# hongsukchoi/Pose2Mesh_RELEASE

Hardware: NVIDIA H100
Metric: SMPL meshes/sec (higher is better)
Workload: dtype f32 (wgmma fp16x3 split, fp32 accumulate)

## Files before the change

include/p2m_b200.h:

```cpp
#ifndef P2M_B200_H_
#define P2M_B200_H_

#include <stddef.h>
#include <stdint.h>

#ifdef __cplusplus
extern "C" {
#endif

typedef struct p2m_model p2m_model_t;
typedef void* p2m_stream_t;

enum p2m_status {
  P2M_OK = 0,
  P2M_ERR_INVALID = 1,
  P2M_ERR_CUDA = 2,
  P2M_ERR_WORKSPACE = 3,
  P2M_ERR_NOGPU = 4
};

enum p2m_precision {
  P2M_PREC_FP32_SIMT = 0,
  P2M_PREC_FP16X3_TC = 1
};
// ... 23 lines not shown
} p2m_params_t;

int p2m_model_create(const p2m_model_desc_t* desc, p2m_model_t** out);
void p2m_model_destroy(p2m_model_t* m);
int p2m_model_num_layers(const p2m_model_t* m);
int p2m_model_layer_info(const p2m_model_t* m, int layer, int32_t out[6]);
int p2m_model_set_precision(p2m_model_t* m, int precision);
int p2m_model_set_profiling(p2m_model_t* m, int enable);
int p2m_model_layer_times_ms(p2m_model_t* m, float* out_ms, int n);
int p2m_debug_kernel_status(p2m_model_t* m, int32_t* out);
int p2m_debug_set_trace(p2m_model_t* m, void* dev_buf);
int p2m_debug_set_fuse_head(p2m_model_t* m, int enable);
int p2m_debug_set_elide_padding(p2m_model_t* m, int enable);
int p2m_debug_set_dedup_padding(p2m_model_t* m, int enable);
int p2m_debug_conv_path(const p2m_model_t* m, int level, int fin, int fout, int32_t out[9]);
int p2m_debug_layer_route(const p2m_model_t* m, int layer, int batch, int need_dx, int32_t out[9]);

typedef struct {
  float* const* z;
  float* const* a;
  float* const* y;
  float* fc_out;
  float* const* g_a;
  float* const* g_z;
  float* const* dx;
  float* fc_dx;
} p2m_capture_t;
int p2m_debug_set_capture(p2m_model_t* m, const p2m_capture_t* capture);

#define P2M_BN_BATCH_UPDATE 0
// ... 350 lines not shown
```

pose2mesh_release_b200/_lib.py:

```python
from __future__ import annotations

import ctypes as C
import os
import threading

import torch

_HERE = os.path.dirname(os.path.abspath(__file__))
LIB_PATH = os.path.join(_HERE, "libp2m_b200.so")

P2M_PREC_FP32_SIMT = 0
P2M_PREC_FP16X3_TC = 1
PRECISIONS = {"fp32": P2M_PREC_FP32_SIMT, "fp16x3": P2M_PREC_FP16X3_TC}


def default_precision() -> int:
    name = os.environ.get("P2M_PRECISION", "fp16x3").strip().lower()
    if name not in PRECISIONS:
        raise RuntimeError(f"P2M_PRECISION={name!r}: expected one of {sorted(PRECISIONS)}")
    return PRECISIONS[name]

c_float_p = C.POINTER(C.c_float)
c_int32_p = C.POINTER(C.c_int32)
c_int64_p = C.POINTER(C.c_int64)
# ... 152 lines not shown
P2M_DTYPE_F64 = 1

P2M_NOISE_NONE = 0
P2M_NOISE_COCO = 1
P2M_NOISE_H36M = 2
P2M_AREA_TIGHT = 0
P2M_AREA_CROP = 1


class H36MError(C.Structure):
    _fields_ = [("mean", C.c_double * 2), ("std", C.c_double * 2), ("weight", C.c_double)]


EXPORTS = [
    "p2m_model_create", "p2m_model_destroy", "p2m_model_num_layers", "p2m_model_layer_info",
    "p2m_model_set_precision", "p2m_debug_kernel_status", "p2m_debug_set_trace", "p2m_debug_set_fuse_head", "p2m_debug_set_elide_padding", "p2m_debug_set_dedup_padding", "p2m_debug_conv_path", "p2m_debug_layer_route", "p2m_debug_set_capture", "p2m_model_set_profiling", "p2m_model_layer_times_ms", "p2m_meshnet_workspace_bytes", "p2m_meshnet_backward_scratch_bytes",
    "p2m_meshnet_forward", "p2m_meshnet_backward", "p2m_meshnet_workspace_bytes_opts", "p2m_meshnet_forward_opts",
    "p2m_meshnet_backward_opts", "p2m_model_set_output_gather", "p2m_meshnet_forward_vertices", "p2m_meshnet_host_io_bytes", "p2m_meshnet_forward_host", "p2m_meshnet_forward_vertices_host",
    "p2m_cheb_conv_workspace_bytes", "p2m_cheb_conv_fwd", "p2m_cheb_conv_bwd", "p2m_graph_match_level", "p2m_posenet_workspace_bytes", "p2m_posenet_forward",
    "p2m_posenet_train_workspace_bytes", "p2m_posenet_train_saved_bytes", "p2m_posenet_train_forward", "p2m_posenet_backward",
    "p2m_posenet_forward_opts", "p2m_posenet_train_forward_opts", "p2m_posenet_backward_opts",
    "p2m_debug_posenet_backward_capture",
    "p2m_regress_joints", "p2m_regress_joints_backward", "p2m_normalize_pose2d", "p2m_mesh_losses", "p2m_coord_loss",
    "p2m_pose2mesh_loss", "p2m_pose2mesh_loss_backward",
    "p2m_rigid_align", "p2m_point_errors", "p2m_fit_camera", "p2m_crop_cam_to_orig",
    "p2m_one_euro_smooth", "p2m_accel_error", "p2m_segment_mean",
    "p2m_nearest_distances", "p2m_align_w_scale", "p2m_pck_accumulate",
    "p2m_render_workspace_bytes", "p2m_render_meshes",
    "p2m_body_model_create", "p2m_body_model_destroy", "p2m_body_model_workspace_bytes", "p2m_body_model_forward",
    "p2m_body_model_backward_workspace_bytes", "p2m_body_model_backward",
    "p2m_camera_frame_workspace_bytes", "p2m_camera_frame_coords", "p2m_h36m_regressors_create",
# ... 32 lines not shown
        lib.p2m_model_set_precision.restype = C.c_int
        lib.p2m_model_set_profiling.argtypes = [vp, C.c_int]
        lib.p2m_model_set_profiling.restype = C.c_int
        lib.p2m_model_layer_times_ms.argtypes = [vp, c_float_p, C.c_int]
        lib.p2m_model_layer_times_ms.restype = C.c_int
        lib.p2m_debug_set_fuse_head.argtypes = [vp, C.c_int]
        lib.p2m_debug_set_fuse_head.restype = C.c_int
        lib.p2m_debug_set_elide_padding.argtypes = [vp, C.c_int]
        lib.p2m_debug_set_elide_padding.restype = C.c_int
        lib.p2m_debug_set_dedup_padding.argtypes = [vp, C.c_int]
        lib.p2m_debug_set_dedup_padding.restype = C.c_int
        lib.p2m_debug_set_trace.argtypes = [vp, vp]
        lib.p2m_debug_set_trace.restype = C.c_int
        lib.p2m_debug_conv_path.argtypes = [vp, C.c_int, C.c_int, C.c_int, c_int32_p]
        lib.p2m_debug_conv_path.restype = C.c_int
        lib.p2m_debug_layer_route.argtypes = [vp, C.c_int, C.c_int, C.c_int, c_int32_p]
        lib.p2m_debug_layer_route.restype = C.c_int
        lib.p2m_debug_set_capture.argtypes = [vp, C.POINTER(Capture)]
        lib.p2m_debug_set_capture.restype = C.c_int
        lib.p2m_debug_kernel_status.argtypes = [vp, c_int32_p]
        lib.p2m_debug_kernel_status.restype = C.c_int
        lib.p2m_meshnet_workspace_bytes.argtypes = [vp, C.c_int, C.c_int]
        lib.p2m_meshnet_workspace_bytes.restype = sz
        lib.p2m_meshnet_backward_scratch_bytes.argtypes = [vp, C.c_int]
        lib.p2m_meshnet_backward_scratch_bytes.restype = sz
        lib.p2m_meshnet_host_io_bytes.argtypes = [vp, C.c_int]
        lib.p2m_meshnet_host_io_bytes.restype = sz
        lib.p2m_meshnet_forward.argtypes = [vp, C.POINTER(Params), vp, vp, C.c_int, C.c_int, vp, sz, vp]
        lib.p2m_meshnet_forward.restype = C.c_int
        lib.p2m_model_set_output_gather.argtypes = [vp, c_int32_p, C.c_int]
# ... 188 lines not shown
```

pose2mesh_release_b200/csrc/cheb_umma.cu:

```cuda
#include <cuda.h>
#include <cuda_fp16.h>
#include <cuda_runtime.h>

#include <algorithm>
#include <climits>
#include <cstring>
#include <vector>

#include "p2m_internal.h"

namespace p2m {

namespace {

constexpr int TILE_M = 128;
constexpr int FC = 32;
constexpr int A_BLOCK_BYTES = TILE_M * 128;
constexpr float W_SCALE = 64.f;
constexpr float W_INV_SCALE = 1.f / 64.f;

struct TileHeader {
  int n_rows;
  int h1;
  int nnz;
// ... 321 lines not shown
template <>
struct ConvRoles<128> {
  static constexpr int threads = NUM_THREADS_W, prod = W_PROD_W, xload = W_XLOAD_W, bload = W_BLOAD_W,
                       epi0 = W_EPI0_W, epi1 = W_EPI1_W;
  static constexpr int regs_launch = REGS_LAUNCH_W, regs_util = REGS_UTIL_W, regs_prod = REGS_PROD_W,
                       regs_epi = REGS_EPI_W;
};

template <int N>
__host__ __device__ constexpr int tile_rows() { return N == 128 ? 64 : TILE_M; }


struct ConvSmem {
  size_t xs, xs_stage, t1s, t1_stage, meta, bars, flags, ep, stage, own, tail, bytes;
};
__host__ __device__ __forceinline__ ConvSmem conv_smem(int N, int NS, int XS, int MODE, int max_h1, int meta_stride) {
  const int tm = N == 128 ? 64 : TILE_M;
  size_t at = 0, sum = 0;
  auto take = [&](size_t bytes) { sum += bytes; at += bytes; return at - bytes; };
  ConvSmem L;
  take((size_t)NS * (tm + N) * 128);
  L.xs_stage = (MODE == 1 && tm == 64) ? 0 : (size_t)tm * FC;
  L.xs = take(XS * L.xs_stage * 4);
  L.t1_stage = MODE == 1 ? (size_t)max_h1 * FC : 0;
  L.t1s = take(XS * L.t1_stage * 4);
  L.meta = take(2 * (size_t)meta_stride);
  L.bars = take(8 * (2 * NS + 2 * XS + 6));
  L.flags = take(16);
  L.ep = take(2 * 4 * N);
  at = (at + 127) & ~(size_t)127;
  L.stage = take(4 * stg_warp_bytes(N));
  L.own = take(4 * 32 * 4);
  L.tail = take(N == 64 ? 64 * 12 * 4 : 4 * 8);
  L.bytes = sum + 128 + 1024 + 32;
  return L;
}

template <int N, int NS, int XS, int MODE>
__device__ __forceinline__ void cheb_conv_body(const KParams& p) {
  static_assert(N == 64 || N == 128, "one warpgroup holds the CTA's 128 x 64 or 64 x 128 accumulator in registers");
  static_assert(NS == 3 || NS == 6, "the producers fill a chunk's three slots back to back");
  using R = ConvRoles<N>;
  constexpr int TM = tile_rows<N>();
  constexpr int NPW = R::prod;
  constexpr int NRG = NPW * 4;
  constexpr int RPT = TM / NRG;
  constexpr int NWG = N == 128 ? 2 : 1;
  static_assert(RPT == 2, "both configurations give a producer thread two tile rows");
  constexpr int H = TM / 64;
  constexpr int ER = 16 * H;
  constexpr bool KT1 = (MODE == 1);
  constexpr bool plain = !KT1;
  constexpr int A_BYTES = TM * 128;
  constexpr int B_BLOCK_BYTES = N * 128;
  constexpr int SLOT_BYTES = A_BYTES + B_BLOCK_BYTES;
  static_assert(NWG * ER == 32 && SLOT_BYTES == (TM + N) * 128, "conv_smem describes this configuration");

  extern __shared__ __align__(1024) unsigned char smem_raw[];
  const ConvSmem L = conv_smem(N, NS, XS, MODE, p.max_h1, p.meta_stride);
  unsigned char* ring = smem_raw;
  float* Xs = reinterpret_cast<float*>(smem_raw + L.xs);
  float* T1s = reinterpret_cast<float*>(smem_raw + L.t1s);
  unsigned char* meta_s = smem_raw + L.meta;
  uint64_t* bars = reinterpret_cast<uint64_t*>(smem_raw + L.bars);
  uint64_t* b_ab_full = bars;
  uint64_t* b_ab_empty = b_ab_full + NS;
  uint64_t* b_x_full = b_ab_empty + NS;
  uint64_t* b_x_empty = b_x_full + XS;
  uint64_t* b_m_full = b_x_empty + XS;
  uint64_t* b_m_empty = b_m_full + 2;
  uint64_t* b_stg_free = b_m_empty + 2;
  uint64_t* b_turn = b_stg_free + 1;
  uint32_t* flags = reinterpret_cast<uint32_t*>(smem_raw + L.flags);
  volatile int* abort_flag = reinterpret_cast<volatile int*>(flags + 1);
  float* ep_mul = reinterpret_cast<float*>(smem_raw + L.ep);
  float* ep_add = ep_mul + N;
  constexpr int EC = 32;
  constexpr int STG_WARP_BYTES = stg_warp_bytes(N);
  unsigned char* epi_stage = smem_raw + L.stage;
  int* own_s = reinterpret_cast<int*>(smem_raw + L.own);
  float* head_w_s = reinterpret_cast<float*>(smem_raw + L.tail);
  uint64_t* b_res = reinterpret_cast<uint64_t*>(head_w_s);

  const int tid = threadIdx.x;
  const int warp = tid >> 5;
  const int lane = tid & 31;
  const int n_chunk = p.fin / FC;
  const int n_use = 3 * n_chunk;

  if (tid == 0) {
    for (int s = 0; s < NS; ++s) {
      mbar_init(smem_u32(b_ab_full + s), p.apack != nullptr ? 1 : NPW + 1);
      mbar_init(smem_u32(b_ab_empty + s), 4);
    }
    for (int s = 0; s < XS; ++s) {
      mbar_init(smem_u32(b_x_full + s), N_XLOAD * 32 + 1);
      mbar_init(smem_u32(b_x_empty + s), 1);
    }
    for (int s = 0; s < 2; ++s) {
      mbar_init(smem_u32(b_m_full + s), 1);
      mbar_init(smem_u32(b_m_empty + s), 1);
    }
    if (N == 128) {
      for (int w = 0; w < 4; ++w) mbar_init(smem_u32(b_res + w), 1);
      mbar_init(smem_u32(b_stg_free), 4);
      mbar_init(smem_u32(b_turn), 4);
    }
    *abort_flag = (smem_u32(ring) & 1023u) ? 1 : 0;
    if (*abort_flag) mbar_timeout(abort_flag, p.status, 100);
    fence_barrier_init();
  }
  const float a_scale = p.a_scale ? *p.a_scale : 1.f;
  const float b_inv = p.b_scale ? 1.f / *p.b_scale : W_INV_SCALE;
  const int ecol0 = (int)blockIdx.y * N;
  for (int n = threadIdx.x; n < N; n += R::threads) {
    const float sc = (p.ep.scale ? p.ep.scale[ecol0 + n] : 1.f) / a_scale;
    const float sh = p.ep.scale ? p.ep.shift[ecol0 + n] : 0.f;
    const float bi = p.ep.bias ? p.ep.bias[ecol0 + n] : 0.f;
    ep_mul[n] = b_inv * sc;
    ep_add[n] = fmaf(bi, p.ep.scale ? p.ep.scale[ecol0 + n] : 1.f, sh);
  }
  if (N == 64 && p.head_z != nullptr)
    for (int i = threadIdx.x; i < 64 * 12; i += R::threads) head_w_s[i] = p.head_wt[i];
  __syncthreads();

  const int mma_g = warp >= R::epi0 ? 0 : (NWG == 2 && warp >= R::epi1 && warp < R::epi1 + 4) ? 1 : -1;
  if (warp >= R::xload && warp < R::epi0) {
  asm volatile("setmaxnreg.dec.sync.aligned.u32 %0;" ::"n"(R::regs_util));
  if (warp >= R::xload && warp < R::xload + N_XLOAD) {
    if (p.apack == nullptr) {
      const int lt = tid - R::xload * 32;
      const int lq = lt & 7, lrg = lt >> 3;
      const int my_tiles = (p.n_tiles - (int)blockIdx.x + (int)gridDim.x - 1) / (int)gridDim.x;
      if (lt == 32 && p.tma) {
        if (plain) asm volatile("prefetch.tensormap [%0];" ::"l"(reinterpret_cast<uint64_t>(&p.tm_x)) : "memory");
// ... 83 lines not shown
            mbar_arrive_expect_tx(smem_u32(b_ab_full + s), B_BLOCK_BYTES + A_BYTES);
            bulk_g2s(smem_u32(ring + s * SLOT_BYTES), p.apack + ((size_t)tile * uses + u) * A_BYTES, A_BYTES,
                     smem_u32(b_ab_full + s));
          } else {
            mbar_arrive_expect_tx(smem_u32(b_ab_full + s), B_BLOCK_BYTES);
          }
          bulk_g2s(smem_u32(ring + s * SLOT_BYTES + A_BYTES), wsl + (size_t)u * (size_t)p.wblock_stride, B_BLOCK_BYTES,
                   smem_u32(b_ab_full + s));
        }
      }
    }
  }
  } else if (mma_g >= 0) {
    asm volatile("setmaxnreg.inc.sync.aligned.u32 %0;" ::"n"(R::regs_epi));
    const int g = mma_g;
    const int wq = warp - (g == 0 ? R::epi0 : R::epi1);
    const int tr = 3 + 2 * g;
    constexpr int CPR = EC / 4;
    constexpr int RPI = 32 / CPR;
    const uint32_t stg = smem_u32(epi_stage) + (uint32_t)wq * STG_WARP_BYTES;
    const int prow = lane / CPR, pc = lane % CPR;
    constexpr int NP = ER / RPI;
    int colk[2];
#pragma unroll
    for (int k = 0; k < 2; ++k) colk[k] = (int)(((uint32_t)pc ^ (uint32_t)((k * RPI + prow) & 7)) << 2);
    const int trow = (lane >> 4) * 64 + wq * 16 + (lane & 15);
    const int uses = plain ? n_chunk : n_use;
    int etn = 0;
    for (int it = g; (int)blockIdx.x + it * (int)gridDim.x < p.n_tiles; it += NWG) {
      const int tile = blockIdx.x + it * gridDim.x;
      const int b = tile / p.P, pat = tile - b * p.P;
      const long long mesh0 = (long long)b * p.V;
      int* own_w = own_s + (g * 4 + wq) * ER;
      {
        int v;
        if (lane >= ER) {
          v = -1;
        } else if (p.own_table) {
          v = __ldg(reinterpret_cast<const int*>(p.meta + (size_t)pat * p.meta_stride + 64) + trow);
        } else {
          v = pat * TM + trow;
          if (v >= p.V) v = -1;
        }
        __syncwarp();
// ... 9 lines not shown
        for (int j = lane; j < ER * lpr; j += 32) {
          const int rr = j / lpr, ln = j - rr * lpr;
          const int vtx = own_w[rr];
          if (vtx >= 0) {
            const long long r = mesh0 + vtx;
            prefetch_l2(p.ep.res + (p.ep.res_unpool ? (r >> 1) : r) * p.ep.res_F + (own_cols ? ecol0 : 0) + ln * 32);
          }
        }
      }
      float acc[2][32];
#pragma unroll
      for (int h = 0; h < 2; ++h)
#pragma unroll
        for (int j = 0; j < 32; ++j) acc[h][j] = 0.f;
      if (wq == 0 && lane == 0) trace_ev(p, tr, etn, 1);
      if (NWG == 2 && it > 0) {
        mbar_wait(smem_u32(b_turn), (uint32_t)(it - 1) & 1u, abort_flag, p.status, 13);
        if (wq == 0 && lane == 0) trace_ev(p, tr, etn, 3);
      }
      uint32_t ucnt = (uint32_t)it * (uint32_t)uses;
      for (int u = 0; u < uses; ++u, ++ucnt) {
        const uint32_t s = ucnt % NS;
        if (wq == 0 && lane == 0) trace_ev(p, tr, etn, 4);
        mbar_wait(smem_u32(b_ab_full + s), (ucnt / NS) & 1, abort_flag, p.status, 6);
        if (wq == 0 && lane == 0) trace_ev(p, tr, etn, 5);
        const uint32_t a0 = smem_u32(ring + s * SLOT_BYTES);
        wg_fence();
        if constexpr (N == 128) {
          const uint64_t da = make_desc_sw128(a0);
          const uint64_t db = make_desc_sw128(a0 + A_BYTES);
          wgmma_m64n128(acc, da + 0, db + 0);
          wgmma_m64n128(acc, da + 2, db + 2);
          wgmma_m64n128(acc, da + 4, db + 0);
          wgmma_m64n128(acc, da + 6, db + 2);
          wgmma_m64n128(acc, da + 0, db + 4);
          wgmma_m64n128(acc, da + 2, db + 6);
        } else {
#pragma unroll
          for (int h = 0; h < 2; ++h) {
            const uint64_t da = make_desc_sw128(a0 + (uint32_t)h * (64 * 128));
            const uint64_t db = make_desc_sw128(a0 + A_BYTES);
            wgmma_m64n64(acc[h], da + 0, db + 0);
            wgmma_m64n64(acc[h], da + 2, db + 2);
            wgmma_m64n64(acc[h], da + 4, db + 0);
            wgmma_m64n64(acc[h], da + 6, db + 2);
            wgmma_m64n64(acc[h], da + 0, db + 4);
            wgmma_m64n64(acc[h], da + 2, db + 6);
          }
        }
        wg_commit();
        wg_wait0();
        __syncwarp();
        if (lane == 0) mbar_arrive(smem_u32(b_ab_empty + s));
      }
      if (NWG == 2 && lane == 0) mbar_arrive(smem_u32(b_turn));
      if (wq == 0 && lane == 0) trace_ev(p, tr, etn, 2);
      auto stage_slab = [&](int cb) {
#pragma unroll
        for (int h = 0; h < H; ++h)
#pragma unroll
          for (int jj = 0; jj < 4; ++jj)
#pragma unroll
            for (int r = 0; r < 2; ++r) {
              const int lr = 16 * h + (lane >> 2) + 8 * r;
              const int cc = 8 * jj + 2 * (lane & 3);
              const int j = 4 * (cb / 8 + jj) + 2 * r;
              sts_f2(stg + lr * (EC * 4) + ((((uint32_t)(cc >> 2)) ^ (uint32_t)(lr & 7)) << 4) + (cc & 3) * 4,
                     acc[h][j], acc[h][j + 1]);
            }
        __syncwarp();
// ... 19 lines not shown
              const float4 w2 = *reinterpret_cast<const float4*>(head_w_s + n * 12 + 8);
              z[0] = fmaf(t, w0.x, z[0]); z[1] = fmaf(t, w0.y, z[1]); z[2] = fmaf(t, w0.z, z[2]); z[3] = fmaf(t, w0.w, z[3]);
              z[4] = fmaf(t, w1.x, z[4]); z[5] = fmaf(t, w1.y, z[5]); z[6] = fmaf(t, w1.z, z[6]); z[7] = fmaf(t, w1.w, z[7]);
              z[8] = fmaf(t, w2.x, z[8]); z[9] = fmaf(t, w2.y, z[9]); z[10] = fmaf(t, w2.z, z[10]); z[11] = fmaf(t, w2.w, z[11]);
            }
          }
          __syncwarp();
        }
        if (own_w[lane] >= 0) {
          float4* zr = reinterpret_cast<float4*>(p.head_z + (mesh0 + own_w[lane]) * 12);
          zr[0] = make_float4(z[0], z[1], z[2], z[3]);
          zr[1] = make_float4(z[4], z[5], z[6], z[7]);
          zr[2] = make_float4(z[8], z[9], z[10], z[11]);
        }
      } else if (N == 128) {
        if (it > 0) mbar_wait(smem_u32(b_stg_free), (uint32_t)(it - 1) & 1u, abort_flag, p.status, 14);
        if (wq == 0 && lane == 0) trace_ev(p, tr, etn, 20);
        const bool res_id = p.ep.res != nullptr && p.res_identity;
        if (res_id) {
          const uint32_t rbar = smem_u32(b_res + wq);
          const int n_valid = __popc(__ballot_sync(0xFFFFFFFFu, lane < ER && own_w[lane] >= 0));
          if (lane == 0) mbar_arrive_expect_tx(rbar, (uint32_t)n_valid * (N * 4));
          __syncwarp();
          if (lane < ER && own_w[lane] >= 0) {
            const long long r = mesh0 + own_w[lane];
            bulk_g2s(stg + lane * STG_ROW_BYTES, p.ep.res + (p.ep.res_unpool ? (r >> 1) : r) * p.ep.res_F + ecol0, N * 4,
                     rbar);
          }
          mbar_wait(rbar, (uint32_t)it & 1u, abort_flag, p.status, 12);
        }
        if (wq == 0 && lane == 0) trace_ev(p, tr, etn, 21);
#pragma unroll
        for (int h = 0; h < 2; ++h)
#pragma unroll
          for (int jg = 0; jg < 8; ++jg) {
            const int n = 64 * h + 8 * jg + 2 * (lane & 3);
            const float2 mu = *reinterpret_cast<const float2*>(ep_mul + n);
            const float2 ad = *reinterpret_cast<const float2*>(ep_add + n);
#pragma unroll
            for (int r = 0; r < 2; ++r) {
              const int j = 4 * jg + 2 * r;
              const uint32_t a = stg + ((lane >> 2) + 8 * r) * STG_ROW_BYTES + n * 4;
              float o0 = fmaf(acc[h][j], mu.x, ad.x), o1 = fmaf(acc[h][j + 1], mu.y, ad.y);
              if (p.ep.relu) {
                o0 = fmaxf(o0, 0.f);
                o1 = fmaxf(o1, 0.f);
              }
              if (res_id) {
                const float2 rv = lds_f2(a);
                o0 += rv.x;
                o1 += rv.y;
              }
              sts_f2(a, o0, o1);
// ... 220 lines not shown
        for (int k = 0; k < 3; ++k) mbar_arrive(smem_u32(b_ab_full + (slot0 + k) % NS));
      }
      if (tid == 0) trace_ev(p, 0, ptn, 7);
      producer_barrier<NPW * 32>();
      if (tid == 0) trace_ev(p, 0, ptn, 8);
      if (tid == 0) mbar_arrive(smem_u32(b_x_empty + xs));
      if (tid == 0 && c == n_chunk - 1) mbar_arrive(smem_u32(b_m_empty + m));
    }
    }
  }
}

template <int N, int NS, int XS, int MODE>
__global__ void __launch_bounds__(NUM_THREADS2, 1) k_cheb_conv_umma(const __grid_constant__ KParams p) {
  static_assert(N == 64, "the 64 x 128 configuration is k_cheb_conv_wide");
  cheb_conv_body<N, NS, XS, MODE>(p);
}
template <int NS, int XS, int MODE>
__global__ void __launch_bounds__(NUM_THREADS_W, 1) k_cheb_conv_wide(const __grid_constant__ KParams p) {
  cheb_conv_body<128, NS, XS, MODE>(p);
}

struct DwParams {
  const float* x;
  int in_unpool;
  int V, P, fin;
  int n_tiles;
  const unsigned char* meta;
  const int* meta_bytes;
  int meta_stride, max_h1;
  const float* g;
  int fout_total, m_off, m_cols;
  int chunk0;
  const float* a_scale;
  float* dw;
// ... 451 lines not shown
    const __half hi = __float2half_rn(w);
    h[e] = (j < 4) ? hi : __float2half_rn(w - __half2float(hi));
  }
  *reinterpret_cast<uint4*>(out + blk * s.rows * 128 + sw128_off(row, j)) = *reinterpret_cast<const uint4*>(h);
}
int launch_pack(const PackSrc& src, long long n_blocks, void* out, cudaStream_t s) {
  const long long total = n_blocks * src.rows * 8;
  k_pack<<<(unsigned)((total + 255) / 256), 256, 0, s>>>(src, total, static_cast<unsigned char*>(out));
  P2M_LAUNCH_OK();
  return P2M_OK;
}

constexpr size_t SMEM_LIMIT = 227 * 1024;
constexpr int CONV_N = 64;
constexpr int WIDE_N = 128;
inline int conv_n(int fout) { return fout % WIDE_N == 0 ? WIDE_N : CONV_N; }
const TileBlobs& conv_tiles(int N, const DevLevel& g, const TileSet* tiles) {
  if (tiles != nullptr) return N == WIDE_N ? tiles->m64 : *tiles;
  return N == WIDE_N ? g.meta64 : g.meta128;
}
struct ConvCfg {
  int ns, xs;
};
ConvCfg conv_cfg(int N, const TileBlobs& t, bool t1_given) {
  for (int ns = N == WIDE_N ? 6 : 3; ns >= 3; ns -= 3)
    for (int xs = 2; xs >= 1; --xs)
      if (conv_smem(N, ns, xs, t1_given, t.max_h1, t.stride).bytes <= SMEM_LIMIT) return {ns, xs};
  return {0, 0};
}

typedef CUresult (*TmapEncodeFn)(CUtensorMap*, CUtensorMapDataType, cuuint32_t, void*, const cuuint64_t*, const cuuint64_t*,
                                 const cuuint32_t*, const cuuint32_t*, CUtensorMapInterleave, CUtensorMapSwizzle,
                                 CUtensorMapL2promotion, CUtensorMapFloatOOBfill);
TmapEncodeFn tmap_encoder() {
  static TmapEncodeFn fn = [] {
    void* f = nullptr;
    cudaDriverEntryPointQueryResult q;
    if (cudaGetDriverEntryPoint("cuTensorMapEncodeTiled", &f, cudaEnableDefault, &q) != cudaSuccess ||
        q != cudaDriverEntryPointSuccess)
      f = nullptr;
    return reinterpret_cast<TmapEncodeFn>(f);
  }();
  return fn;
}
bool make_row_tmap(CUtensorMap* tm, const float* base, long long rows, int fin, int box_rows) {
  TmapEncodeFn enc = tmap_encoder();
  if (enc == nullptr || (reinterpret_cast<uintptr_t>(base) & 15u) != 0) return false;
  const cuuint64_t dims[2] = {(cuuint64_t)fin, (cuuint64_t)rows};
  const cuuint64_t strides[1] = {(cuuint64_t)fin * 4};
  const cuuint32_t box[2] = {(cuuint32_t)FC, (cuuint32_t)box_rows};
  const cuuint32_t estr[2] = {1, 1};
  return enc(tm, CU_TENSOR_MAP_DATA_TYPE_FLOAT32, 2, const_cast<float*>(base), dims, strides, box, estr,
             CU_TENSOR_MAP_INTERLEAVE_NONE, CU_TENSOR_MAP_SWIZZLE_NONE, CU_TENSOR_MAP_L2_PROMOTION_L2_128B,
             CU_TENSOR_MAP_FLOAT_OOB_FILL_NONE) == CUDA_SUCCESS;
}

template <int N, int NS, int XS, int MODE>
constexpr auto conv_kernel() {
  if constexpr (N == WIDE_N) return k_cheb_conv_wide<NS, XS, MODE>;
  else return k_cheb_conv_umma<N, NS, XS, MODE>;
}
template <int N, int NS, int XS, int MODE>
int check_launch_regs() {
  static int state = 0;
  if (state == 0) {
    cudaFuncAttributes fa;
    P2M_CUDA_OK(cudaFuncGetAttributes(&fa, conv_kernel<N, NS, XS, MODE>()));
    state = (fa.numRegs == ConvRoles<N>::regs_launch) ? 1 : -1;
  }
  if (state < 0) {
    set_error(N == WIDE_N
                  ? "k_cheb_conv_wide was compiled with a register count other than the one its setmaxnreg split assumes"
                  : "k_cheb_conv_umma was compiled with a register count other than the one its setmaxnreg split assumes");
    return P2M_ERR_CUDA;
  }
  return P2M_OK;
}

template <int N, int NS, int XS>
int launch_cfg(const UmmaConvArgs& a, int* status, const float* zero_row, int sm_count, cudaStream_t s) {
  constexpr int TM = tile_rows<N>();
  const DevLevel& g = *a.g;
  const TileBlobs& t = conv_tiles(N, g, a.tiles);
  const size_t smem = conv_smem(N, NS, XS, !a.plain, t.max_h1, t.stride).bytes;
  auto kern = a.plain ? conv_kernel<N, NS, XS, 0>() : conv_kernel<N, NS, XS, 1>();
  P2M_CUDA_OK(cudaFuncSetAttribute(kern, cudaFuncAttributeMaxDynamicSharedMemorySize, (int)smem));
  P2M_TRY((a.plain ? check_launch_regs<N, NS, XS, 0>() : check_launch_regs<N, NS, XS, 1>()));
  KParams p;
  p.x = a.x;
  p.in_unpool = a.in_unpool;
  p.V = g.V;
  p.P = t.n_pattern;
  p.fin = a.fin;
  p.meta = t.meta;
  p.meta_bytes = t.bytes;
  p.meta_stride = t.stride;
  p.max_h1 = t.max_h1;
  p.own_table = a.tiles != nullptr ? 1 : 0;
  p.n_tiles = a.batch * p.P;
  p.wpack = static_cast<const unsigned char*>(a.wpack);
  p.apack = nullptr;
  p.wslice_bytes = (long long)N * 128;
  p.wblock_stride = (long long)a.fout * 128;
  p.zero_row = zero_row;
  p.ep = to_dev(a.ep);
  p.res_identity = (a.ep.res != nullptr && a.ep.res_F == a.fout) ? 1 : 0;
  p.y = a.y;
  p.t1 = a.t1;
  p.a_scale = a.a_scale;
  p.b_scale = nullptr;
  p.ldy = a.ldy > 0 ? a.ldy : a.fout;
  p.y_col0 = a.y_col0;
  p.status = status;
  p.trace = a.trace;
  p.head_wt = a.fout == 64 ? a.head_wt : nullptr;
  p.head_z = a.fout == 64 ? a.head_z : nullptr;
  if (N == WIDE_N) {
// ... 1 lines not shown
    const bool res_ok = !p.res_identity || ((reinterpret_cast<uintptr_t>(p.ep.res) & 15u) == 0 && (p.ep.res_F * 4) % 16 == 0);
    if (!y_ok || !res_ok) {
      set_error("umma_conv: the 128-column epilogue needs 16-byte aligned output and identity-residual rows");
      return P2M_ERR_INVALID;
    }
  }
  p.tma = 0;
  std::memset(&p.tm_x, 0, sizeof(p.tm_x));
  std::memset(&p.tm_t1, 0, sizeof(p.tm_t1));
  if (a.tiles == nullptr && g.V % TILE_M == 0) {
    const long long rows = (long long)a.batch * g.V;
    bool ok = make_row_tmap(&p.tm_x, a.x, a.in_unpool ? rows / 2 : rows, a.fin, a.in_unpool ? TM / 2 : TM);
    if (ok && a.t1 != nullptr) ok = make_row_tmap(&p.tm_t1, a.t1, rows, a.fin, TM);
    p.tma = ok ? 1 : 0;
  }
  const int n_slices = a.fout / N;
  const dim3 grid(std::min(p.n_tiles, std::max(1, sm_count / n_slices)), n_slices);
  kern<<<grid, ConvRoles<N>::threads, smem, s>>>(p);
  P2M_LAUNCH_OK();
  return P2M_OK;
}

int launch_n(const UmmaConvArgs& a, int* status, const float* zero_row, int sm_count, cudaStream_t s) {
  const int N = conv_n(a.fout);
  const ConvCfg c = conv_cfg(N, conv_tiles(N, *a.g, a.tiles), !a.plain);
  if (c.ns == 0) {
    set_error("umma_conv: tile family does not fit shared memory");
    return P2M_ERR_INVALID;
  }
  if (N == CONV_N)
    return c.xs == 2 ? launch_cfg<CONV_N, 3, 2>(a, status, zero_row, sm_count, s)
                     : launch_cfg<CONV_N, 3, 1>(a, status, zero_row, sm_count, s);
  if (c.ns == 6)
    return c.xs == 2 ? launch_cfg<WIDE_N, 6, 2>(a, status, zero_row, sm_count, s)
                     : launch_cfg<WIDE_N, 6, 1>(a, status, zero_row, sm_count, s);
  return c.xs == 2 ? launch_cfg<WIDE_N, 3, 2>(a, status, zero_row, sm_count, s)
                   : launch_cfg<WIDE_N, 3, 1>(a, status, zero_row, sm_count, s);
}

}

namespace {
void balance_store_halves(std::vector<unsigned short>* ord) {
  std::vector<unsigned short> q0, q1;
// ... 244 lines not shown
  P2M_LAUNCH_OK();
  return P2M_OK;
}

bool umma_conv_supported(const DevLevel& g, int fin, int fout) {
  if (g.meta128.n_pattern <= 0) return false;
  if (fin % FC != 0 || fin < FC || fin > 256) return false;
  if (g.meta128.max_h1 > 256) return false;
  if (fout != 64 && fout != 128 && fout != 256) return false;
  const int N = conv_n(fout);
  const TileBlobs& t = conv_tiles(N, g, nullptr);
  return t.n_pattern > 0 && conv_smem(N, 3, 1, 1, t.max_h1, t.stride).bytes <= SMEM_LIMIT &&
         conv_smem(N, 3, 1, 0, t.max_h1, t.stride).bytes <= SMEM_LIMIT;
}

int umma_conv_x_stages(const DevLevel& g, int fout, bool plain) {
  const int N = conv_n(fout);
  return conv_cfg(N, conv_tiles(N, g, nullptr), !plain).xs;
}
bool umma_tma_rows(const DevLevel& g) { return g.V % TILE_M == 0 && tmap_encoder() != nullptr; }

size_t umma_plain_pack_bytes(int N, int K) { return (size_t)(K / FC) * N * 128; }

static size_t gemm_x_image_bytes(int M, int K) { return (size_t)((M + TILE_M - 1) / TILE_M) * (K / FC) * A_BLOCK_BYTES; }
size_t umma_gemm_apack_bytes(int M, int K) { return gemm_x_image_bytes(M, K) + 128; }
size_t umma_gemm_wpack_bytes(int N, int K) { return (size_t)(K / FC) * N * 128; }
bool umma_gemm_supported(int M, int N, int K) { return M > 0 && K >= FC && K % FC == 0 && N >= 64 && N % 64 == 0; }

namespace {
template <int N>
int launch_gemm_cfg(KParams p, int n_slices, int sm_count, cudaStream_t s) {
  constexpr int NS = 3;
  const size_t smem = conv_smem(N, NS, 1, 0, 0, 0).bytes;
// ... 86 lines not shown
```

pose2mesh_release_b200/csrc/p2m_api.cu:

```cuda
#include <cuda_runtime.h>

#include <algorithm>
#include <cmath>
#include <cstring>
#include <memory>
#include <string>
#include <tuple>
#include <vector>

#include "p2m_internal.h"

namespace p2m {

static thread_local std::string g_error;
static thread_local int64_t g_launches = 0;
void set_error(const std::string& msg) { g_error = msg; }
void count_launch(int n) { g_launches += n; }

int arrays_device(const char* where, std::initializer_list<const void*> arrays, int* dev) {
  int found = -1;
  for (const void* p : arrays) {
    if (!p) continue;
    cudaPointerAttributes attr;
    if (cudaPointerGetAttributes(&attr, p) != cudaSuccess ||
// ... 756 lines not shown
  return P2M_OK;
}
int p2m_debug_set_dedup_padding(p2m_model_t* m, int enable) {
  if (!m) return P2M_ERR_INVALID;
  m->dedup_padding = enable ? 1 : 0;
  return P2M_OK;
}
int p2m_debug_conv_path(const p2m_model_t* m, int level, int fin, int fout, int32_t out[9]) {
  if (!m || !out || level < 0 || level >= (int)m->levels.size() || fin <= 0 || fout <= 0) {
    set_error("debug_conv_path: bad argument");
    return P2M_ERR_INVALID;
  }
  const DevLevel& g = m->levels[level];
  const ConvRoute r = conv_route(m, level, fin, fout, 1, false);
  out[0] = r.tc;
  out[1] = r.tc ? umma_conv_x_stages(g, fout, false) : 0;
  out[2] = r.tc_dw;
  out[3] = r.tc_dw ? umma_dw_x_stages(g) : 0;
  out[4] = r.tc_dt;
  out[5] = r.tc_dt ? umma_conv_x_stages(g, fin, true) : 0;
  out[6] = (g.meta128.n_pattern > 0 && umma_tma_rows(g)) ? 1 : 0;
  out[7] = g.meta128.max_h1;
  out[8] = g.n_iso;
  return P2M_OK;
}

int p2m_debug_layer_route(const p2m_model_t* m, int layer, int batch, int need_dx, int32_t out[9]) {
  if (!m || !out || layer < 0 || layer >= (int)m->layers.size() || batch <= 0) {
    set_error("debug_layer_route: bad argument");
    return P2M_ERR_INVALID;
  }
  const Layer& L = m->layers[layer];
  int b = 0;
  while (m->blocks[b].first_layer + m->blocks[b].n_layers <= layer) ++b;
  const ConvRoute f = conv_route(m, L.level, L.fin, L.fout, batch, true);
  const ConvRoute r = backward_route(m, layer, batch, layer > 0 || need_dx);
  out[0] = f.tc;
  out[1] = f.elide;
// ... 661 lines not shown
```

pose2mesh_release_b200/csrc/p2m_internal.h:

```cpp
#pragma once
#include <cuda_runtime.h>
#include <stdint.h>

#include <initializer_list>
#include <string>
#include <vector>

#include "../../include/p2m_b200.h"

namespace p2m {

void set_error(const std::string& msg);
void count_launch(int n = 1);

#define P2M_CUDA_OK(expr)                                                                     \
  do {                                                                                        \
    cudaError_t _e = (expr);                                                                  \
    if (_e != cudaSuccess) {                                                                  \
      p2m::set_error(std::string(#expr) + " failed: " + cudaGetErrorString(_e) + " (" +        \
                     __FILE__ + ":" + std::to_string(__LINE__) + ")");                        \
      return P2M_ERR_CUDA;                                                                    \
    }                                                                                         \
  } while (0)

// ... 332 lines not shown
  const float* t1 = nullptr;
  int plain = 0;
  const float* a_scale = nullptr;
  long long ldy = 0;
  int y_col0 = 0;
  const float* head_wt = nullptr;
  float* head_z = nullptr;
  const TileSet* tiles = nullptr;
  long long* trace = nullptr;
};
int build_umma_level_meta(const int* rowptr, const int* colidx, const float* val, int V, DevLevel* out,
                          std::vector<void*>* owned);
int build_tileset(const std::vector<int>& rows, const int* rowptr, const int* colidx, const float* val, int V,
                  TileSet* ts, std::vector<void*>* owned);
bool umma_conv_supported(const DevLevel& g, int fin, int fout);
int umma_conv_x_stages(const DevLevel& g, int fout, bool plain);
int umma_dw_x_stages(const DevLevel& g);
bool umma_tma_rows(const DevLevel& g);
constexpr int WPACK_ALL = -1, WPACK_COMBINED = -2;
size_t umma_wpack_bytes(int fin, int fout);
size_t umma_plain_pack_bytes(int N, int K);
int launch_umma_pack_weights(const float* W, int fin, int fout, bool transposed, int order, float c, void* wpack,
                             cudaStream_t s);
int launch_absmax_scale(const float* x, long long n, float* scale_out, cudaStream_t s, int headroom_log2 = 0);
int launch_absmax_finish(unsigned int* amax, float* scale_out, cudaStream_t s, int headroom_log2 = 0);
int launch_scale_by(const float* x, long long n, const float* scale, int invert, float mul, float* y, cudaStream_t s);
int launch_rescaled_epilogue(const Epilogue& ep, const float* w_scale, float w_packed, int n, float* out_scale,
                             float* out_shift, cudaStream_t s);
bool umma_dw_supported(const DevLevel& g, int gathered_width, int plain_width);
int launch_umma_dw(const DevLevel& g, int batch, const float* gathered, int in_unpool, int gathered_width,
                   const float* t1, const float* plain, int g_unpool, int plain_width, int swap, const float* a_scale,
// ... 21 lines not shown
```

Measured before the change: 12570.

## Add 64x256 pair-column conv tiling sharing A tiles across both MMA warpgroups

For 256→256 Chebyshev convs with a given T1, the wide conv kernel gets a 256-column configuration. Both MMA warpgroups consume the same A slot, each with its own 128-column half of B, instead of alternating tiles. This halves the number of column slices, so X/T1 gathering and A staging are reused across twice the output columns. The cost is a larger B ring per slot, which forces fewer pipeline stages (NS=3), and per-CTA work that is serialized differently. A debug query reporting the chosen tiling is also added.

```diff
diff --git a/include/p2m_b200.h b/include/p2m_b200.h
--- a/include/p2m_b200.h
+++ b/include/p2m_b200.h
@@ -61,6 +61,7 @@
 int p2m_debug_set_elide_padding(p2m_model_t* m, int enable);
 int p2m_debug_set_dedup_padding(p2m_model_t* m, int enable);
 int p2m_debug_conv_path(const p2m_model_t* m, int level, int fin, int fout, int32_t out[9]);
+int p2m_debug_conv_tiling(const p2m_model_t* m, int level, int fin, int fout, int32_t out[3]);
 int p2m_debug_layer_route(const p2m_model_t* m, int layer, int batch, int need_dx, int32_t out[9]);
 
 typedef struct {
diff --git a/pose2mesh_release_b200/_lib.py b/pose2mesh_release_b200/_lib.py
--- a/pose2mesh_release_b200/_lib.py
+++ b/pose2mesh_release_b200/_lib.py
@@ -190,7 +190,7 @@
 
 EXPORTS = [
     "p2m_model_create", "p2m_model_destroy", "p2m_model_num_layers", "p2m_model_layer_info",
-    "p2m_model_set_precision", "p2m_debug_kernel_status", "p2m_debug_set_trace", "p2m_debug_set_fuse_head", "p2m_debug_set_elide_padding", "p2m_debug_set_dedup_padding", "p2m_debug_conv_path", "p2m_debug_layer_route", "p2m_debug_set_capture", "p2m_model_set_profiling", "p2m_model_layer_times_ms", "p2m_meshnet_workspace_bytes", "p2m_meshnet_backward_scratch_bytes",
+    "p2m_model_set_precision", "p2m_debug_kernel_status", "p2m_debug_set_trace", "p2m_debug_set_fuse_head", "p2m_debug_set_elide_padding", "p2m_debug_set_dedup_padding", "p2m_debug_conv_path", "p2m_debug_conv_tiling", "p2m_debug_layer_route", "p2m_debug_set_capture", "p2m_model_set_profiling", "p2m_model_layer_times_ms", "p2m_meshnet_workspace_bytes", "p2m_meshnet_backward_scratch_bytes",
     "p2m_meshnet_forward", "p2m_meshnet_backward", "p2m_meshnet_workspace_bytes_opts", "p2m_meshnet_forward_opts",
     "p2m_meshnet_backward_opts", "p2m_model_set_output_gather", "p2m_meshnet_forward_vertices", "p2m_meshnet_host_io_bytes", "p2m_meshnet_forward_host", "p2m_meshnet_forward_vertices_host",
     "p2m_cheb_conv_workspace_bytes", "p2m_cheb_conv_fwd", "p2m_cheb_conv_bwd", "p2m_graph_match_level", "p2m_posenet_workspace_bytes", "p2m_posenet_forward",
@@ -253,6 +253,8 @@
         lib.p2m_debug_set_trace.restype = C.c_int
         lib.p2m_debug_conv_path.argtypes = [vp, C.c_int, C.c_int, C.c_int, c_int32_p]
         lib.p2m_debug_conv_path.restype = C.c_int
+        lib.p2m_debug_conv_tiling.argtypes = [vp, C.c_int, C.c_int, C.c_int, c_int32_p]
+        lib.p2m_debug_conv_tiling.restype = C.c_int
         lib.p2m_debug_layer_route.argtypes = [vp, C.c_int, C.c_int, C.c_int, c_int32_p]
         lib.p2m_debug_layer_route.restype = C.c_int
         lib.p2m_debug_set_capture.argtypes = [vp, C.POINTER(Capture)]
diff --git a/pose2mesh_release_b200/csrc/cheb_umma.cu b/pose2mesh_release_b200/csrc/cheb_umma.cu
--- a/pose2mesh_release_b200/csrc/cheb_umma.cu
+++ b/pose2mesh_release_b200/csrc/cheb_umma.cu
@@ -359,12 +359,13 @@
 struct ConvSmem {
   size_t xs, xs_stage, t1s, t1_stage, meta, bars, flags, ep, stage, own, tail, bytes;
 };
-__host__ __device__ __forceinline__ ConvSmem conv_smem(int N, int NS, int XS, int MODE, int max_h1, int meta_stride) {
+__host__ __device__ __forceinline__ ConvSmem conv_smem(int NC, int NS, int XS, int MODE, int max_h1, int meta_stride) {
+  const int N = NC == 64 ? 64 : 128;
   const int tm = N == 128 ? 64 : TILE_M;
   size_t at = 0, sum = 0;
   auto take = [&](size_t bytes) { sum += bytes; at += bytes; return at - bytes; };
   ConvSmem L;
-  take((size_t)NS * (tm + N) * 128);
+  take((size_t)NS * (tm + NC) * 128);
   L.xs_stage = (MODE == 1 && tm == 64) ? 0 : (size_t)tm * FC;
   L.xs = take(XS * L.xs_stage * 4);
   L.t1_stage = MODE == 1 ? (size_t)max_h1 * FC : 0;
@@ -372,7 +373,7 @@
   L.meta = take(2 * (size_t)meta_stride);
   L.bars = take(8 * (2 * NS + 2 * XS + 6));
   L.flags = take(16);
-  L.ep = take(2 * 4 * N);
+  L.ep = take(2 * 4 * NC);
   at = (at + 127) & ~(size_t)127;
   L.stage = take(4 * stg_warp_bytes(N));
   L.own = take(4 * 32 * 4);
@@ -381,9 +382,11 @@
   return L;
 }
 
-template <int N, int NS, int XS, int MODE>
+template <int N, int NC, int NS, int XS, int MODE>
 __device__ __forceinline__ void cheb_conv_body(const KParams& p) {
   static_assert(N == 64 || N == 128, "one warpgroup holds the CTA's 128 x 64 or 64 x 128 accumulator in registers");
+  static_assert(NC == N || (N == 128 && NC == 2 * N && MODE == 1),
+                "64 x 256: both MMA warpgroups of the 64 x 128 layout, T1-given convs only (conv_cols)");
   static_assert(NS == 3 || NS == 6, "the producers fill a chunk's three slots back to back");
   using R = ConvRoles<N>;
   constexpr int TM = tile_rows<N>();
@@ -391,18 +394,19 @@
   constexpr int NRG = NPW * 4;
   constexpr int RPT = TM / NRG;
   constexpr int NWG = N == 128 ? 2 : 1;
+  constexpr bool COLS = NC != N;
   static_assert(RPT == 2, "both configurations give a producer thread two tile rows");
   constexpr int H = TM / 64;
   constexpr int ER = 16 * H;
   constexpr bool KT1 = (MODE == 1);
   constexpr bool plain = !KT1;
   constexpr int A_BYTES = TM * 128;
-  constexpr int B_BLOCK_BYTES = N * 128;
+  constexpr int B_BLOCK_BYTES = NC * 128;
   constexpr int SLOT_BYTES = A_BYTES + B_BLOCK_BYTES;
-  static_assert(NWG * ER == 32 && SLOT_BYTES == (TM + N) * 128, "conv_smem describes this configuration");
+  static_assert(NWG * ER == 32 && SLOT_BYTES == (TM + NC) * 128, "conv_smem describes this configuration");
 
   extern __shared__ __align__(1024) unsigned char smem_raw[];
-  const ConvSmem L = conv_smem(N, NS, XS, MODE, p.max_h1, p.meta_stride);
+  const ConvSmem L = conv_smem(NC, NS, XS, MODE, p.max_h1, p.meta_stride);
   unsigned char* ring = smem_raw;
   float* Xs = reinterpret_cast<float*>(smem_raw + L.xs);
   float* T1s = reinterpret_cast<float*>(smem_raw + L.t1s);
@@ -419,7 +423,7 @@
   uint32_t* flags = reinterpret_cast<uint32_t*>(smem_raw + L.flags);
   volatile int* abort_flag = reinterpret_cast<volatile int*>(flags + 1);
   float* ep_mul = reinterpret_cast<float*>(smem_raw + L.ep);
-  float* ep_add = ep_mul + N;
+  float* ep_add = ep_mul + NC;
   constexpr int EC = 32;
   constexpr int STG_WARP_BYTES = stg_warp_bytes(N);
   unsigned char* epi_stage = smem_raw + L.stage;
@@ -436,7 +440,7 @@
   if (tid == 0) {
     for (int s = 0; s < NS; ++s) {
       mbar_init(smem_u32(b_ab_full + s), p.apack != nullptr ? 1 : NPW + 1);
-      mbar_init(smem_u32(b_ab_empty + s), 4);
+      mbar_init(smem_u32(b_ab_empty + s), COLS ? 8 : 4);
     }
     for (int s = 0; s < XS; ++s) {
       mbar_init(smem_u32(b_x_full + s), N_XLOAD * 32 + 1);
@@ -457,13 +461,13 @@
   }
   const float a_scale = p.a_scale ? *p.a_scale : 1.f;
   const float b_inv = p.b_scale ? 1.f / *p.b_scale : W_INV_SCALE;
-  const int ecol0 = (int)blockIdx.y * N;
-  for (int n = threadIdx.x; n < N; n += R::threads) {
-    const float sc = (p.ep.scale ? p.ep.scale[ecol0 + n] : 1.f) / a_scale;
-    const float sh = p.ep.scale ? p.ep.shift[ecol0 + n] : 0.f;
-    const float bi = p.ep.bias ? p.ep.bias[ecol0 + n] : 0.f;
+  const int ccol0 = (int)blockIdx.y * NC;
+  for (int n = threadIdx.x; n < NC; n += R::threads) {
+    const float sc = (p.ep.scale ? p.ep.scale[ccol0 + n] : 1.f) / a_scale;
+    const float sh = p.ep.scale ? p.ep.shift[ccol0 + n] : 0.f;
+    const float bi = p.ep.bias ? p.ep.bias[ccol0 + n] : 0.f;
     ep_mul[n] = b_inv * sc;
-    ep_add[n] = fmaf(bi, p.ep.scale ? p.ep.scale[ecol0 + n] : 1.f, sh);
+    ep_add[n] = fmaf(bi, p.ep.scale ? p.ep.scale[ccol0 + n] : 1.f, sh);
   }
   if (N == 64 && p.head_z != nullptr)
     for (int i = threadIdx.x; i < 64 * 12; i += R::threads) head_w_s[i] = p.head_wt[i];
@@ -577,6 +581,9 @@
   } else if (mma_g >= 0) {
     asm volatile("setmaxnreg.inc.sync.aligned.u32 %0;" ::"n"(R::regs_epi));
     const int g = mma_g;
+    const int ecol0 = ccol0 + (COLS ? g * N : 0);
+    const float* ep_mul_g = ep_mul + (COLS ? g * N : 0);
+    const float* ep_add_g = ep_add + (COLS ? g * N : 0);
     const int wq = warp - (g == 0 ? R::epi0 : R::epi1);
     const int tr = 3 + 2 * g;
     constexpr int CPR = EC / 4;
@@ -590,7 +597,8 @@
     const int trow = (lane >> 4) * 64 + wq * 16 + (lane & 15);
     const int uses = plain ? n_chunk : n_use;
     int etn = 0;
-    for (int it = g; (int)blockIdx.x + it * (int)gridDim.x < p.n_tiles; it += NWG) {
+    for (int it = COLS ? 0 : g; (int)blockIdx.x + it * (int)gridDim.x < p.n_tiles; it += COLS ? 1 : NWG) {
+      const int e = COLS ? 2 * it + g : it;
       const int tile = blockIdx.x + it * gridDim.x;
       const int b = tile / p.P, pat = tile - b * p.P;
       const long long mesh0 = (long long)b * p.V;
@@ -630,7 +638,7 @@
 #pragma unroll
         for (int j = 0; j < 32; ++j) acc[h][j] = 0.f;
       if (wq == 0 && lane == 0) trace_ev(p, tr, etn, 1);
-      if (NWG == 2 && it > 0) {
+      if (NWG == 2 && !COLS && it > 0) {
         mbar_wait(smem_u32(b_turn), (uint32_t)(it - 1) & 1u, abort_flag, p.status, 13);
         if (wq == 0 && lane == 0) trace_ev(p, tr, etn, 3);
       }
@@ -644,7 +652,7 @@
         wg_fence();
         if constexpr (N == 128) {
           const uint64_t da = make_desc_sw128(a0);
-          const uint64_t db = make_desc_sw128(a0 + A_BYTES);
+          const uint64_t db = make_desc_sw128(a0 + A_BYTES + (COLS ? (uint32_t)g * (N * 128) : 0u));
           wgmma_m64n128(acc, da + 0, db + 0);
           wgmma_m64n128(acc, da + 2, db + 2);
           wgmma_m64n128(acc, da + 4, db + 0);
@@ -669,7 +677,7 @@
         __syncwarp();
         if (lane == 0) mbar_arrive(smem_u32(b_ab_empty + s));
       }
-      if (NWG == 2 && lane == 0) mbar_arrive(smem_u32(b_turn));
+      if (NWG == 2 && !COLS && lane == 0) mbar_arrive(smem_u32(b_turn));
       if (wq == 0 && lane == 0) trace_ev(p, tr, etn, 2);
       auto stage_slab = [&](int cb) {
 #pragma unroll
@@ -719,7 +727,7 @@
           zr[2] = make_float4(z[8], z[9], z[10], z[11]);
         }
       } else if (N == 128) {
-        if (it > 0) mbar_wait(smem_u32(b_stg_free), (uint32_t)(it - 1) & 1u, abort_flag, p.status, 14);
+        if (e > 0) mbar_wait(smem_u32(b_stg_free), (uint32_t)(e - 1) & 1u, abort_flag, p.status, 14);
         if (wq == 0 && lane == 0) trace_ev(p, tr, etn, 20);
         const bool res_id = p.ep.res != nullptr && p.res_identity;
         if (res_id) {
@@ -732,7 +740,7 @@
             bulk_g2s(stg + lane * STG_ROW_BYTES, p.ep.res + (p.ep.res_unpool ? (r >> 1) : r) * p.ep.res_F + ecol0, N * 4,
                      rbar);
           }
-          mbar_wait(rbar, (uint32_t)it & 1u, abort_flag, p.status, 12);
+          mbar_wait(rbar, (uint32_t)e & 1u, abort_flag, p.status, 12);
         }
         if (wq == 0 && lane == 0) trace_ev(p, tr, etn, 21);
 #pragma unroll
@@ -740,8 +748,8 @@
 #pragma unroll
           for (int jg = 0; jg < 8; ++jg) {
             const int n = 64 * h + 8 * jg + 2 * (lane & 3);
-            const float2 mu = *reinterpret_cast<const float2*>(ep_mul + n);
-            const float2 ad = *reinterpret_cast<const float2*>(ep_add + n);
+            const float2 mu = *reinterpret_cast<const float2*>(ep_mul_g + n);
+            const float2 ad = *reinterpret_cast<const float2*>(ep_add_g + n);
 #pragma unroll
             for (int r = 0; r < 2; ++r) {
               const int j = 4 * jg + 2 * r;
@@ -992,11 +1000,11 @@
 template <int N, int NS, int XS, int MODE>
 __global__ void __launch_bounds__(NUM_THREADS2, 1) k_cheb_conv_umma(const __grid_constant__ KParams p) {
   static_assert(N == 64, "the 64 x 128 configuration is k_cheb_conv_wide");
-  cheb_conv_body<N, NS, XS, MODE>(p);
-}
-template <int NS, int XS, int MODE>
+  cheb_conv_body<N, N, NS, XS, MODE>(p);
+}
+template <int NC, int NS, int XS, int MODE>
 __global__ void __launch_bounds__(NUM_THREADS_W, 1) k_cheb_conv_wide(const __grid_constant__ KParams p) {
-  cheb_conv_body<128, NS, XS, MODE>(p);
+  cheb_conv_body<128, NC, NS, XS, MODE>(p);
 }
 
 struct DwParams {
@@ -1478,6 +1486,7 @@
 constexpr size_t SMEM_LIMIT = 227 * 1024;
 constexpr int CONV_N = 64;
 constexpr int WIDE_N = 128;
+constexpr int PAIR_N = 256;
 inline int conv_n(int fout) { return fout % WIDE_N == 0 ? WIDE_N : CONV_N; }
 const TileBlobs& conv_tiles(int N, const DevLevel& g, const TileSet* tiles) {
   if (tiles != nullptr) return N == WIDE_N ? tiles->m64 : *tiles;
@@ -1486,11 +1495,15 @@
 struct ConvCfg {
   int ns, xs;
 };
-ConvCfg conv_cfg(int N, const TileBlobs& t, bool t1_given) {
-  for (int ns = N == WIDE_N ? 6 : 3; ns >= 3; ns -= 3)
+ConvCfg conv_cfg(int NC, const TileBlobs& t, bool t1_given) {
+  for (int ns = NC == WIDE_N ? 6 : 3; ns >= 3; ns -= 3)
     for (int xs = 2; xs >= 1; --xs)
-      if (conv_smem(N, ns, xs, t1_given, t.max_h1, t.stride).bytes <= SMEM_LIMIT) return {ns, xs};
+      if (conv_smem(NC, ns, xs, t1_given, t.max_h1, t.stride).bytes <= SMEM_LIMIT) return {ns, xs};
   return {0, 0};
+}
+int conv_cols(int fin, int fout, const TileBlobs& t, bool t1_given) {
+  const bool pair = fout == PAIR_N && fin == PAIR_N && t1_given && conv_cfg(PAIR_N, t, true).ns > 0;
+  return pair ? PAIR_N : conv_n(fout);
 }
 
 typedef CUresult (*TmapEncodeFn)(CUtensorMap*, CUtensorMapDataType, cuuint32_t, void*, const cuuint64_t*, const cuuint64_t*,
@@ -1519,17 +1532,18 @@
              CU_TENSOR_MAP_FLOAT_OOB_FILL_NONE) == CUDA_SUCCESS;
 }
 
-template <int N, int NS, int XS, int MODE>
+template <int NC, int NS, int XS, int MODE>
 constexpr auto conv_kernel() {
-  if constexpr (N == WIDE_N) return k_cheb_conv_wide<NS, XS, MODE>;
-  else return k_cheb_conv_umma<N, NS, XS, MODE>;
-}
-template <int N, int NS, int XS, int MODE>
+  if constexpr (NC != CONV_N) return k_cheb_conv_wide<NC, NS, XS, MODE>;
+  else return k_cheb_conv_umma<NC, NS, XS, MODE>;
+}
+template <int NC, int NS, int XS, int MODE>
 int check_launch_regs() {
+  constexpr int N = NC == CONV_N ? CONV_N : WIDE_N;
   static int state = 0;
   if (state == 0) {
     cudaFuncAttributes fa;
-    P2M_CUDA_OK(cudaFuncGetAttributes(&fa, conv_kernel<N, NS, XS, MODE>()));
+    P2M_CUDA_OK(cudaFuncGetAttributes(&fa, conv_kernel<NC, NS, XS, MODE>()));
     state = (fa.numRegs == ConvRoles<N>::regs_launch) ? 1 : -1;
   }
   if (state < 0) {
@@ -1541,15 +1555,17 @@
   return P2M_OK;
 }
 
-template <int N, int NS, int XS>
+template <int NC, int NS, int XS>
 int launch_cfg(const UmmaConvArgs& a, int* status, const float* zero_row, int sm_count, cudaStream_t s) {
+  constexpr int N = NC == CONV_N ? CONV_N : WIDE_N;
   constexpr int TM = tile_rows<N>();
   const DevLevel& g = *a.g;
   const TileBlobs& t = conv_tiles(N, g, a.tiles);
-  const size_t smem = conv_smem(N, NS, XS, !a.plain, t.max_h1, t.stride).bytes;
-  auto kern = a.plain ? conv_kernel<N, NS, XS, 0>() : conv_kernel<N, NS, XS, 1>();
+  const size_t smem = conv_smem(NC, NS, XS, !a.plain, t.max_h1, t.stride).bytes;
+  constexpr int M0 = NC == PAIR_N ? 1 : 0;
+  auto kern = a.plain ? conv_kernel<NC, NS, XS, M0>() : conv_kernel<NC, NS, XS, 1>();
   P2M_CUDA_OK(cudaFuncSetAttribute(kern, cudaFuncAttributeMaxDynamicSharedMemorySize, (int)smem));
-  P2M_TRY((a.plain ? check_launch_regs<N, NS, XS, 0>() : check_launch_regs<N, NS, XS, 1>()));
+  P2M_TRY((a.plain ? check_launch_regs<NC, NS, XS, M0>() : check_launch_regs<NC, NS, XS, 1>()));
   KParams p;
   p.x = a.x;
   p.in_unpool = a.in_unpool;
@@ -1564,7 +1580,7 @@
   p.n_tiles = a.batch * p.P;
   p.wpack = static_cast<const unsigned char*>(a.wpack);
   p.apack = nullptr;
-  p.wslice_bytes = (long long)N * 128;
+  p.wslice_bytes = (long long)NC * 128;
   p.wblock_stride = (long long)a.fout * 128;
   p.zero_row = zero_row;
   p.ep = to_dev(a.ep);
@@ -1596,7 +1612,7 @@
     if (ok && a.t1 != nullptr) ok = make_row_tmap(&p.tm_t1, a.t1, rows, a.fin, TM);
     p.tma = ok ? 1 : 0;
   }
-  const int n_slices = a.fout / N;
+  const int n_slices = a.fout / NC;
   const dim3 grid(std::min(p.n_tiles, std::max(1, sm_count / n_slices)), n_slices);
   kern<<<grid, ConvRoles<N>::threads, smem, s>>>(p);
   P2M_LAUNCH_OK();
@@ -1605,11 +1621,16 @@
 
 int launch_n(const UmmaConvArgs& a, int* status, const float* zero_row, int sm_count, cudaStream_t s) {
   const int N = conv_n(a.fout);
-  const ConvCfg c = conv_cfg(N, conv_tiles(N, *a.g, a.tiles), !a.plain);
+  const TileBlobs& t = conv_tiles(N, *a.g, a.tiles);
+  const int NC = conv_cols(a.fin, a.fout, t, !a.plain);
+  const ConvCfg c = conv_cfg(NC, t, !a.plain);
   if (c.ns == 0) {
     set_error("umma_conv: tile family does not fit shared memory");
     return P2M_ERR_INVALID;
   }
+  if (NC == PAIR_N)
+    return c.xs == 2 ? launch_cfg<PAIR_N, 3, 2>(a, status, zero_row, sm_count, s)
+                     : launch_cfg<PAIR_N, 3, 1>(a, status, zero_row, sm_count, s);
   if (N == CONV_N)
     return c.xs == 2 ? launch_cfg<CONV_N, 3, 2>(a, status, zero_row, sm_count, s)
                      : launch_cfg<CONV_N, 3, 1>(a, status, zero_row, sm_count, s);
@@ -1884,9 +1905,15 @@
          conv_smem(N, 3, 1, 0, t.max_h1, t.stride).bytes <= SMEM_LIMIT;
 }
 
-int umma_conv_x_stages(const DevLevel& g, int fout, bool plain) {
+int umma_conv_x_stages(const DevLevel& g, int fin, int fout, bool plain) {
+  return umma_conv_tiling(g, fin, fout, plain).xs;
+}
+UmmaConvTiling umma_conv_tiling(const DevLevel& g, int fin, int fout, bool plain) {
   const int N = conv_n(fout);
-  return conv_cfg(N, conv_tiles(N, g, nullptr), !plain).xs;
+  const TileBlobs& t = conv_tiles(N, g, nullptr);
+  const int NC = conv_cols(fin, fout, t, !plain);
+  const ConvCfg c = conv_cfg(NC, t, !plain);
+  return {NC, c.ns, c.xs};
 }
 bool umma_tma_rows(const DevLevel& g) { return g.V % TILE_M == 0 && tmap_encoder() != nullptr; }
 
diff --git a/pose2mesh_release_b200/csrc/p2m_api.cu b/pose2mesh_release_b200/csrc/p2m_api.cu
--- a/pose2mesh_release_b200/csrc/p2m_api.cu
+++ b/pose2mesh_release_b200/csrc/p2m_api.cu
@@ -794,14 +794,28 @@
   const DevLevel& g = m->levels[level];
   const ConvRoute r = conv_route(m, level, fin, fout, 1, false);
   out[0] = r.tc;
-  out[1] = r.tc ? umma_conv_x_stages(g, fout, false) : 0;
+  out[1] = r.tc ? umma_conv_x_stages(g, fin, fout, false) : 0;
   out[2] = r.tc_dw;
   out[3] = r.tc_dw ? umma_dw_x_stages(g) : 0;
   out[4] = r.tc_dt;
-  out[5] = r.tc_dt ? umma_conv_x_stages(g, fin, true) : 0;
+  out[5] = r.tc_dt ? umma_conv_x_stages(g, fout, fin, true) : 0;
   out[6] = (g.meta128.n_pattern > 0 && umma_tma_rows(g)) ? 1 : 0;
   out[7] = g.meta128.max_h1;
   out[8] = g.n_iso;
+  return P2M_OK;
+}
+
+int p2m_debug_conv_tiling(const p2m_model_t* m, int level, int fin, int fout, int32_t out[3]) {
+  if (!m || !out || level < 0 || level >= (int)m->levels.size() || fin <= 0 || fout <= 0) {
+    set_error("debug_conv_tiling: bad argument");
+    return P2M_ERR_INVALID;
+  }
+  const DevLevel& g = m->levels[level];
+  const UmmaConvTiling t = conv_route(m, level, fin, fout, 1, false).tc ? umma_conv_tiling(g, fin, fout, false)
+                                                                        : UmmaConvTiling{0, 0, 0};
+  out[0] = t.cols;
+  out[1] = t.ns;
+  out[2] = t.xs;
   return P2M_OK;
 }
 
diff --git a/pose2mesh_release_b200/csrc/p2m_internal.h b/pose2mesh_release_b200/csrc/p2m_internal.h
--- a/pose2mesh_release_b200/csrc/p2m_internal.h
+++ b/pose2mesh_release_b200/csrc/p2m_internal.h
@@ -370,7 +370,11 @@
 int build_tileset(const std::vector<int>& rows, const int* rowptr, const int* colidx, const float* val, int V,
                   TileSet* ts, std::vector<void*>* owned);
 bool umma_conv_supported(const DevLevel& g, int fin, int fout);
-int umma_conv_x_stages(const DevLevel& g, int fout, bool plain);
+int umma_conv_x_stages(const DevLevel& g, int fin, int fout, bool plain);
+struct UmmaConvTiling {
+  int cols, ns, xs;
+};
+UmmaConvTiling umma_conv_tiling(const DevLevel& g, int fin, int fout, bool plain);
 int umma_dw_x_stages(const DevLevel& g);
 bool umma_tma_rows(const DevLevel& g);
 constexpr int WPACK_ALL = -1, WPACK_COMBINED = -2;
```

Result: faster. 13240, median of 6 (+5.3%).
